# infil00p/openbts-ttsou

Measured on AMD Instinct MI355X. Metric: Mbursts/s (156.25-sym @ 4 sps) demod+detect, higher is better.
Workload: dtype f32

## Files before the change

### openbts-ttsou_amd/csrc/trxsig_corr.h

```cpp
#pragma once
#include "trxsig_dev.h"

namespace {

template <int SPS>
struct CorrGeom {
  static constexpr int NL = 36 * SPS;
  static constexpr int NC = (NL + 15) / 16;
  static constexpr int FRONT = 8 * SPS;
  static constexpr int WPAD0 = NC * 16 + 15 * SPS + 1;
  static constexpr int WPAD = ((WPAD0 + 15) / 32) * 32 + 16;
  static constexpr int H = (5 * SPS + 1 > 12) ? 5 * SPS + 1 : 12;
  static constexpr int NS = 2 * H + 1;
  static constexpr int NE = 20 * SPS;
  static constexpr int NEQ = (NE + 15) / 16;
  static constexpr int NPAIR = (NS + 2) / 2;
};
template <typename T>
__device__ __forceinline__ T &rec_slot(T *rec, int Bpad, int s, int b) { return rec[2 * ((size_t)(s >> 1) * Bpad + b) + (s & 1)]; }

template <int N>
__device__ __forceinline__ float add_row_shl(float acc, float v) {
  float r;
  if (N == 0) asm volatile("v_add_f32 %0, %1, %2" : "=v"(r) : "v"(v), "v"(acc));
  else asm volatile("v_add_f32_dpp %0, %1, %2 row_shl:%3 row_mask:0xf bank_mask:0xf bound_ctrl:1"
                    : "=v"(r) : "v"(v), "v"(acc), "n"(N));
  return r;
}
template <int SPS, int I>
__device__ __forceinline__ float energy_chain_step(float acc, const float (&nrm)[CorrGeom<SPS>::NEQ]) {
  if constexpr (I < CorrGeom<SPS>::NE) {
    acc = add_row_shl<I % 16>(acc, nrm[I / 16]);
    return energy_chain_step<SPS, I + 1>(acc, nrm);
  } else {
    return acc;
  }
}
template <int SPS, int I>
__device__ __forceinline__ float energy_chain(float acc, const float (&nrm)[CorrGeom<SPS>::NEQ]) {
  asm volatile("s_nop 1");
  return energy_chain_step<SPS, I>(acc, nrm);
}

template <int SPS>
struct CorrIn {
  typedef CorrGeom<SPS> G;
  static constexpr int NW = (CorrGeom<SPS>::NL + 15) / 16;
  cx w[NW];
  cx e[CorrGeom<SPS>::NEQ];
  int b;
  bool live, good;
  __device__ __forceinline__ void stage_window(cx *W, int r) const {
#pragma unroll
    for (int i = 0; i < NW; i++) {
      const int q = r + 16 * i;
      if (q < G::NL) W[G::FRONT + q] = w[i];
    }
  }
  __device__ __forceinline__ void stage_norms(float *ef, int r) const {
#pragma unroll
    for (int q = 0; q < G::NEQ; q++) {
      const int i = r + 16 * q;
      if (i < G::NE) ef[i] = norm2(e[q]);
    }
  }
};

template <int SPS>
__device__ __forceinline__ void corr_issue(CorrIn<SPS> &in, int b, int B, int r, const cx *__restrict__ samples,
                                           const int32_t *__restrict__ offset, const int32_t *__restrict__ length) {
  typedef CorrGeom<SPS> G;
  in.b = b;
  in.live = b < B;
  int off = 0, len = 0;
  if (in.live) { off = offset[b]; len = length[b]; }
  in.good = in.live && (off >= 0) && (len >= 92 * SPS) && (len <= 157 * SPS) && (len % SPS == 0);
  const cx *x = samples + (in.good ? off : 0);
#pragma unroll
  for (int i = 0; i < CorrIn<SPS>::NW; i++) {
    const int q = r + 16 * i;
    in.w[i] = (in.good && q < G::NL) ? x[56 * SPS + q] : mk(0, 0);
  }
#pragma unroll
  for (int q = 0; q < G::NEQ; q++) {
    const int i = r + 16 * q;
    in.e[q] = (in.good && i < G::NE) ? x[i] : mk(0, 0);
  }
}

template <int SPS, bool REC, bool EFIRST = false, unsigned TAPCLS = TRX_TAPS_GENERIC, typename IN = CorrIn<SPS>>
__device__ __forceinline__ void corr_round(const IN &in, cx *W, float4 *E, int lane, int r, const cx (&tap)[16],
                                           cx *__restrict__ rec, int Bpad, int &M_out, float &energy_out) {
  typedef CorrGeom<SPS> G;
  auto stage_norms = [&] { in.stage_norms(reinterpret_cast<float *>(E), r); };
  auto sum_norms = [&] {
    float energy = 0.0f;
#pragma unroll
    for (int i4 = 0; i4 < (G::NE + 3) / 4; i4++) {
      const float4 e = E[i4];
      energy = energy + e.x;
      if (4 * i4 + 1 < G::NE) energy = energy + e.y;
      if (4 * i4 + 2 < G::NE) energy = energy + e.z;
      if (4 * i4 + 3 < G::NE) energy = energy + e.w;
    }
    return energy;
  };
  float energy = 0.0f;
  if (EFIRST) {
    stage_norms();
    wave_lds_fence();
    energy = sum_norms();
    asm volatile("" : "+v"(energy));
    wave_lds_fence();
  }
  for (int q = r; q < G::FRONT; q += 16) W[q] = mk(0, 0);
  for (int q = G::FRONT + G::NL + r; q < G::WPAD; q += 16) W[q] = mk(0, 0);
  in.stage_window(W, r);
  if (!EFIRST) stage_norms();
  wave_lds_fence();
  if (!EFIRST) energy = sum_norms();

  float bestP = 0.0f;
  int bestT = -1;
  cx cval[G::NC];
  constexpr int CG = (SPS == 4) ? TRX_CORR_CG : 1;
  constexpr int UPC = 16 / SPS;
  constexpr int NU = UPC * (CG - 1) + 16;
#pragma unroll
  for (int c0 = 0; c0 < G::NC; c0 += CG) {
    cx sv[NU];
#pragma unroll
    for (int u = 0; u < NU; u++) sv[u] = W[r + 16 * c0 + SPS * u];
#pragma unroll
    for (int cc = 0; cc < CG; cc++) {
      if (c0 + cc < G::NC) {
        cx acc = mk(0, 0);
#pragma unroll
        for (int k = 15; k >= 0; k--) acc = cadd(acc, cmul_tap(sv[UPC * cc + k], tap[k], (TAPCLS >> (2 * k)) & 3));
        cval[c0 + cc] = acc;
      }
    }
  }
  wave_lds_fence();
#pragma unroll
  for (int c = 0; c < G::NC; c++) {
    const int t = r + 16 * c;
    if (t < G::NL) {
      W[t] = cval[c];
      const float p = norm2(cval[c]);
      if (p > bestP) { bestP = p; bestT = t; }
    }
  }
#pragma unroll
  for (int m = 1; m < 16; m <<= 1) {
    const float oP = __shfl_xor(bestP, m, 64);
    const int oT = __shfl_xor(bestT, m, 64);
    const bool take = (oP > bestP) || (oP == bestP && oT >= 0 && (bestT < 0 || oT < bestT));
    if (take) { bestP = oP; bestT = oT; }
  }
  wave_lds_fence();

  M_out = bestT;
  energy_out = energy;
  if (REC && in.live) {
    const int M = bestT;
    auto slot = [&](int s) {
      cx v = mk(0, 0);
      if (s < G::NS) {
        const int lag = M - G::H + s;
        if (lag >= 0 && lag < G::NL) v = W[lag];
      } else if (s == G::NS) {
        v = mk(__int_as_float(in.good ? M : -2), energy);
      }
      return v;
    };
    for (int j = r; j < G::NPAIR; j += 16) {
      const cx a = slot(2 * j), c = slot(2 * j + 1);
      reinterpret_cast<float4 *>(rec)[(size_t)j * Bpad + in.b] = make_float4(a.r, a.i, c.r, c.i);
    }
  }
  wave_lds_fence();
  (void)lane;
}


inline unsigned tap_classes(const TrxTables *hT, int tsc) {
  unsigned m = 0;
  for (int k = 0; k < 16; k++) {
    const trx_c32 a = hT->mid_ctap[tsc][k];
    const unsigned c = (a.r == 1.0f || a.r == -1.0f) ? 1u : ((a.i == 1.0f || a.i == -1.0f) ? 2u : 0u);
    m |= c << (2 * k);
  }
  return m;
}

}
```

### openbts-ttsou_amd/csrc/trxsig_dev.h

```cpp
#pragma once
#include <hip/hip_runtime.h>
#include <hip/hip_fp16.h>
#include <stdint.h>

#include <type_traits>

#include "trxsig_tables.h"
#include "trxsig_launch.h"

#ifndef TRX_CORR_CG
#define TRX_CORR_CG 3
#endif
#ifndef TRX_CORR_WPS
#define TRX_CORR_WPS 1
#endif
#ifndef TRX_CORR_ROUNDS
#define TRX_CORR_ROUNDS 1
#endif
#ifndef TRX_DEMOD_WAVES
#define TRX_DEMOD_WAVES 4
#endif

namespace {

typedef trx_c32 cx;

__device__ __forceinline__ cx mk(float r, float i) { cx z; z.r = r; z.i = i; return z; }
__device__ __forceinline__ cx cmul(cx x, cx a) { return mk(x.r * a.r - x.i * a.i, x.r * a.i + x.i * a.r); }
__device__ __forceinline__ cx cmulr(cx x, float a) { return mk(x.r * a, x.i * a); }
__device__ __forceinline__ cx cadd(cx x, cx a) { return mk(x.r + a.r, x.i + a.i); }
__device__ __forceinline__ float norm2(cx x) { return x.i * x.i + x.r * x.r; }
__device__ __forceinline__ cx cinv(cx x) { float n = norm2(x); return mk(x.r / n, -x.i / n); }
__device__ __forceinline__ cx cdiv(cx x, cx a) { return cmul(x, cinv(a)); }

template <int CTRL>
__device__ __forceinline__ float dpp_f(float v) {
  return __int_as_float(__builtin_amdgcn_update_dpp(0, __float_as_int(v), CTRL, 0xf, 0xf, true));
}
template <int CTRL>
__device__ __forceinline__ int dpp_i(int v) { return __builtin_amdgcn_update_dpp(0, v, CTRL, 0xf, 0xf, true); }
__device__ __forceinline__ float wave_sum_any_order(float v) {
  v += dpp_f<0xB1>(v);
  v += dpp_f<0x4E>(v);
  v += dpp_f<0x141>(v);
  v += dpp_f<0x140>(v);
  const float r0 = __int_as_float(__builtin_amdgcn_readlane(__float_as_int(v), 0));
  const float r1 = __int_as_float(__builtin_amdgcn_readlane(__float_as_int(v), 16));
  const float r2 = __int_as_float(__builtin_amdgcn_readlane(__float_as_int(v), 32));
  const float r3 = __int_as_float(__builtin_amdgcn_readlane(__float_as_int(v), 48));
  return ((r0 + r1) + r2) + r3;
}
__device__ __forceinline__ void argmax_take(float &P, int &T, float oP, int oT) {
  const bool take = (oP > P) || (oP == P && oT >= 0 && (T < 0 || oT < T));
  P = take ? oP : P;
  T = take ? oT : T;
}
__device__ __forceinline__ void wave_argmax(float &P, int &T) {
  argmax_take(P, T, dpp_f<0xB1>(P), dpp_i<0xB1>(T));
  argmax_take(P, T, dpp_f<0x4E>(P), dpp_i<0x4E>(T));
  argmax_take(P, T, dpp_f<0x141>(P), dpp_i<0x141>(T));
  argmax_take(P, T, dpp_f<0x140>(P), dpp_i<0x140>(T));
  float bp = __int_as_float(__builtin_amdgcn_readlane(__float_as_int(P), 0));
  int bt = __builtin_amdgcn_readlane(T, 0);
#pragma unroll
  for (int r = 16; r < 64; r += 16)
    argmax_take(bp, bt, __int_as_float(__builtin_amdgcn_readlane(__float_as_int(P), r)), __builtin_amdgcn_readlane(T, r));
  P = bp; T = bt;
}

typedef float v2f __attribute__((ext_vector_type(2)));
__device__ __forceinline__ v2f pk(cx z) { v2f v = {z.r, z.i}; return v; }
__device__ __forceinline__ v2f pk_cmul(v2f x, v2f a) {
  v2f p, q, r;
  asm("v_pk_mul_f32 %0, %1, %2 op_sel_hi:[0,1]" : "=v"(p) : "v"(x), "v"(a));
  asm("v_pk_mul_f32 %0, %1, %2 op_sel:[1,1] op_sel_hi:[1,0]" : "=v"(q) : "v"(x), "v"(a));
  asm("v_pk_add_f32 %0, %1, %2 neg_lo:[0,1]" : "=v"(r) : "v"(p), "v"(q));
  return r;
}
__device__ __forceinline__ v2f pk_mul(v2f x, v2f a) {
  v2f r;
  asm("v_pk_mul_f32 %0, %1, %2" : "=v"(r) : "v"(x), "v"(a));
  return r;
}
template <int HI>
__device__ __forceinline__ v2f pk_mul_tap(v2f x, v2f t) {
  v2f r;
  if (HI) asm("v_pk_mul_f32 %0, %1, %2 op_sel:[0,1] op_sel_hi:[1,1]" : "=v"(r) : "v"(x), "v"(t));
  else asm("v_pk_mul_f32 %0, %1, %2 op_sel_hi:[1,0]" : "=v"(r) : "v"(x), "v"(t));
  return r;
}
__device__ __forceinline__ v2f pk_csub(v2f x, v2f a) {
  v2f r;
  asm("v_pk_add_f32 %0, %1, %2 neg_lo:[0,1] neg_hi:[0,1]" : "=v"(r) : "v"(x), "v"(a));
  return r;
}
__device__ __forceinline__ cx unpk(v2f v) { return mk(v.x, v.y); }
__device__ __forceinline__ v2f pk_cadd(v2f x, v2f a) {
  v2f r;
  asm("v_pk_add_f32 %0, %1, %2" : "=v"(r) : "v"(x), "v"(a));
  return r;
}

struct SmpC32 {
  static constexpr int kBytes = 8;
  static __device__ __forceinline__ cx ld(const void *base, long long i) { return reinterpret_cast<const cx *>(base)[i]; }
  typedef cx raw_t;
  static __device__ __forceinline__ raw_t ldraw(const void *base, long long i) { return reinterpret_cast<const cx *>(base)[i]; }
  static __device__ __forceinline__ raw_t zero() { return mk(0, 0); }
  static __device__ __forceinline__ cx widen(raw_t r) { return r; }
  static __device__ __forceinline__ float4 ld2(const void *base, long long first, int q) {
    return reinterpret_cast<const float4 *>(reinterpret_cast<const cx *>(base) + first)[q];
  }
};
struct SmpF16 {
  static constexpr int kBytes = 4;
  static __device__ __forceinline__ cx ld(const void *base, long long i) {
    const float2 v = __half22float2(reinterpret_cast<const __half2 *>(base)[i]);
    return mk(v.x, v.y);
  }
  typedef unsigned raw_t;
  static __device__ __forceinline__ raw_t ldraw(const void *base, long long i) { return reinterpret_cast<const unsigned *>(base)[i]; }
  static __device__ __forceinline__ raw_t zero() { return 0u; }
  static __device__ __forceinline__ cx widen(raw_t r) {
    const float2 v = __half22float2(*reinterpret_cast<const __half2 *>(&r));
    return mk(v.x, v.y);
  }
  static __device__ __forceinline__ float4 ld2(const void *base, long long first, int q) {
    const uint2 u = reinterpret_cast<const uint2 *>(reinterpret_cast<const __half2 *>(base) + first)[q];
    const float2 a = __half22float2(*reinterpret_cast<const __half2 *>(&u.x)), b = __half22float2(*reinterpret_cast<const __half2 *>(&u.y));
    return make_float4(a.x, a.y, b.x, b.y);
  }
};

struct TapArg { float v[32]; };

#define TRX_TAPS_GENERIC 0u
template <int SPS> struct TapPattern {
  static constexpr unsigned value = (SPS == 4) ? 0x19999999u : 0x99999999u;
};
__device__ __forceinline__ float fma_steer(float a, float b, float c) {
  float r;
  asm("v_fma_f32 %0, %1, %2, %3 ; steering" : "=v"(r) : "v"(a), "v"(b), "v"(c));
  return r;
}
__device__ __forceinline__ float fma_steer_s(float a, float b_sgpr, float c) {
  float r;
  asm("v_fma_f32 %0, %1, %2, %3 ; steering" : "=v"(r) : "v"(a), "s"(b_sgpr), "v"(c));
  return r;
}
__device__ __forceinline__ cx cmul_tap(cx x, cx a, int cls) {
  if (cls == 1) {
    const float p = x.i * a.i, q = x.r * a.i;
    cx z;
    asm("v_fma_f32 %0, %2, %4, -%5 ; exact-product\n\tv_fma_f32 %1, %3, %4, %6 ; exact-product"
        : "=&v"(z.r), "=v"(z.i) : "v"(x.r), "v"(x.i), "s"(a.r), "v"(p), "v"(q));
    return z;
  }
  if (cls == 2) {
    const float p = x.r * a.r, q = x.i * a.r;
    cx z;
    asm("v_fma_f32 %0, %3, -%4, %5 ; exact-product\n\tv_fma_f32 %1, %2, %4, %6 ; exact-product"
        : "=&v"(z.r), "=v"(z.i) : "v"(x.r), "v"(x.i), "s"(a.i), "v"(p), "v"(q));
    return z;
  }
  return cmul(x, a);
}

// ... 49 lines not shown
```

### openbts-ttsou_amd/csrc/trxsig_normal.hip

```cpp
#include "trxsig_bisect.h"
#include "trxsig_corr.h"
#include "trxsig_demod.h"
#include "trxsig_rxgen.h"

#ifndef TRX_RXC_WPS
#define TRX_RXC_WPS 1
#endif
#ifndef TRX_RXD_WPS
#define TRX_RXD_WPS 1
#endif

namespace {

template <int SPS, unsigned TAPCLS>
__global__ __launch_bounds__(256, TRX_CORR_WPS) void k_tsc_corr(const TrxTables *__restrict__ T,
                                                  const cx *__restrict__ samples,
                                                  const int32_t *__restrict__ offset,
                                                  const int32_t *__restrict__ length, int B, TapArg taps,
                                                  cx *__restrict__ rec, int Bpad) {
  typedef CorrGeom<SPS> G;
  static_assert(8 * G::WPAD >= 4 * G::NE, "the energy norms are staged in the row itself");
  __shared__ __attribute__((aligned(16))) cx rows[16][G::WPAD];
  (void)T;
  const int lane = threadIdx.x & 63, wave = threadIdx.x >> 6;
  const int row = lane >> 4, r = lane & 15;
  const int slot = wave * 4 + row;

  cx tap[16];
#pragma unroll
  for (int k = 0; k < 16; k++) tap[k] = mk(taps.v[2 * k], taps.v[2 * k + 1]);

  typedef CorrIn<SPS> In;
  In in[TRX_CORR_ROUNDS];
#pragma unroll
  for (int i = 0; i < TRX_CORR_ROUNDS; i++)
    corr_issue<SPS>(in[i], (blockIdx.x * TRX_CORR_ROUNDS + i) * 16 + slot, B, r, samples, offset, length);
#pragma unroll
  for (int i = 0; i < TRX_CORR_ROUNDS; i++) {
    int M;
    float energy;
    corr_round<SPS, true, true, TAPCLS, In>(in[i], rows[slot], reinterpret_cast<float4 *>(rows[slot]), lane, r, tap, rec, Bpad, M, energy);
  }
}


#ifdef TRX_TUNING_BUILD
template <int SPS>
__global__ __launch_bounds__(64) void k_tsc_peak(const TrxTables *__restrict__ T,
                                                 const cx *__restrict__ rec, int Bpad, int B, int tsc,
                                                 float detect_thresh, float energy_thresh,
                                                 uint8_t *__restrict__ flags, cx *__restrict__ amp_out,
                                                 float *__restrict__ toa_out,
                                                 float *__restrict__ avgpwr_out) {
  typedef CorrGeom<SPS> G;
  __shared__ cx loc[26][64];
  __shared__ float pw[G::NS][64];
  const int lane = threadIdx.x;
  const int b = blockIdx.x * 64 + lane;
  const bool live = b < B;
  const int bb = live ? b : B - 1;

  const cx meta = rec_slot(rec, Bpad, G::NS, bb);
  const int M = __float_as_int(meta.r);
  const float energy = meta.i;
  const bool good = M != -2;
#pragma unroll
  for (int s = 0; s < G::NS; s++) {
    const cx v = rec_slot(rec, Bpad, s, bb);
    pw[s][lane] = norm2(v);
    const int j = s - (G::H - 12);
    if (j >= 0 && j < 24) {
      const int lag = M - 12 + j;
      loc[j][lane] = (lag > G::NL - 2) ? mk(0, 0) : v;
    }
  }
  loc[24][lane] = mk(0, 0);
  loc[25][lane] = mk(0, 0);

  float peakIx;
  const cx peak = peak_bisect<64>(T->sinc_grid, loc, lane, M, &peakIx);

  float toa = peakIx;
  cx amp = peak;
  bool detected = false;
  const bool energy_ok = good && (energy_thresh < 0.0f ||
                                  energy / (float)(unsigned)G::NE > energy_thresh * energy_thresh);
  if (!(toa < 0.0f) && !(toa > (float)G::NL) && good) {
    const int p = (int)rintf(toa);
    float valley = 0.0f;
    int numRms = 0;
#pragma unroll
    for (int i = 2 * SPS; i <= 5 * SPS; i++) {
      const int lo = p - i, hi = p + i;
      int slo = lo - M + G::H, shi = hi - M + G::H;
      slo = slo < 0 ? 0 : slo; shi = shi > G::NS - 1 ? G::NS - 1 : shi;
      const float vlo = pw[slo][lane], vhi = pw[shi][lane];
      if (lo >= 0) { valley += vlo; numRms++; }
      if (hi < G::NL) { valley += vhi; numRms++; }
    }
    if (numRms < 2) {
      amp = mk(0, 0);
    } else {
      const float RMS = (float)((double)sqrtf(valley / (float)numRms) + 0.00001);
      const float peakToMean = sqrtf(norm2(amp)) / RMS;
      amp = cdiv(amp, T->mid_gain[tsc]);
      toa = toa - T->mid_toa[tsc];
      toa = toa - (float)((66 - 56) * SPS);
      detected = peakToMean > detect_thresh;
    }
  } else {
    amp = mk(0, 0);
  }
  if (!energy_ok) { amp = mk(0, 0); toa = 0.0f; detected = false; }

  if (live) {
    uint8_t fl = 0;
    if (!good) fl = TRXSIG_F_BADLEN;
    else fl = (energy_ok ? TRXSIG_F_ENERGY : 0) | (detected ? TRXSIG_F_DETECT : 0);
    flags[b] = fl;
    amp_out[b] = amp;
    toa_out[b] = toa;
    if (avgpwr_out) avgpwr_out[b] = good ? energy / (float)(unsigned)G::NE : 0.0f;
  }
}


template <int SPS>
struct Peak8Geom {
  typedef CorrGeom<SPS> G;
  static constexpr int NV = 2 * (3 * SPS + 1);
  static constexpr int O_PW = 26 * 2;
  static constexpr int O_V = O_PW + ((G::NS + 3) & ~3);
  static constexpr int STRIDE = O_V + ((NV + 3) & ~3);
};

template <int SPS>
__global__ __launch_bounds__(256, 8) void k_tsc_peak8(const TrxTables *__restrict__ T, const cx *__restrict__ rec, int Bpad,
                                                   int B, cx gain_inv, float mid_toa, float detect_thresh,
                                                   float energy_thresh, uint8_t *__restrict__ flags,
                                                   cx *__restrict__ amp_out, float *__restrict__ toa_out,
                                                   float *__restrict__ avgpwr_out) {
  typedef CorrGeom<SPS> G;
  typedef Peak8Geom<SPS> P8;
  __shared__ __attribute__((aligned(16))) float stab[32][24];
  __shared__ __attribute__((aligned(16))) float scratch[32][P8::STRIDE];
  {
    float tv[3];
#pragma unroll
    for (int k = 0; k < 3; k++) { const int ix = threadIdx.x * 3 + k; tv[k] = T->sinc_grid[16 * (ix / 24)][ix % 24]; }
#pragma unroll
    for (int k = 0; k < 3; k++) { const int ix = threadIdx.x * 3 + k; stab[ix / 24][ix % 24] = tv[k]; }
  }
  const int lane = threadIdx.x & 63;
  const int r = lane & 7;
  const int slot = threadIdx.x >> 3;
  const int b = blockIdx.x * 32 + slot;
  const bool live = b < B;
  const int bb = live ? b : B - 1;
  float *S = scratch[slot];
  cx *loc = reinterpret_cast<cx *>(S);
  float *pw = S + P8::O_PW, *V = S + P8::O_V;

  const cx meta = rec_slot(rec, Bpad, G::NS, bb);
  const int M = __float_as_int(meta.r);
  const float energy = meta.i;
  const bool good = M != -2;
#pragma unroll
  for (int s0 = 0; s0 < G::NS; s0 += 8) {
    const int sl = s0 + r;
    if (sl < G::NS) {
      const cx v = rec_slot(rec, Bpad, sl, bb);
      pw[sl] = norm2(v);
      const int j = sl - (G::H - 12);
      if (j >= 0 && j < 24) loc[j] = (M - 12 + j > G::NL - 2) ? mk(0, 0) : v;
    }
  }
  if (r < 2) loc[24 + r] = mk(0, 0);
  __syncthreads();

  int e = 0;
  asm volatile("" : "+v"(e));
  bool active = true;
  cx peak = mk(0, 0);
  {
    const int rel2 = kFusedRel2.v[r], rel1 = kFusedRel1.v[r];
#pragma unroll
    for (int st = 0; st < 4; st++) {
      const int inc_last = 128 >> (2 * st);
      const int el = e + (rel2 >> 2) * inc_last;
      float srow[24];
      if (st < 3) {
        const float4 *rw = reinterpret_cast<const float4 *>(stab[(el & 511) >> 4]);
#pragma unroll
        for (int q = 0; q < 6; q++) {
          const float4 t4 = rw[q];
          srow[4 * q] = t4.x; srow[4 * q + 1] = t4.y; srow[4 * q + 2] = t4.z; srow[4 * q + 3] = t4.w;
        }
      } else {
        fused_row(T, el, srow);
      }
      const cx pt = fused_point(loc, el, rel2 & 3, srow);
      fused_decide<8, 2, false>(pt, lane, 2 * inc_last, e, active, peak);
    }
    {
      float srow[24];
      fused_row(T, e, srow);
      const cx pt = fused_point(loc, e, rel1 & 3, srow);
      fused_decide<8, 1, false>(pt, lane, 1, e, active, peak);
    }
    float srow[24];
    fused_row(T, e, srow);
    peak = fused_point(loc, e, 1, srow);
    asm volatile("" : "+v"(peak.r), "+v"(peak.i));
  }
  cx amp;
  float toa;
  bool detected, energy_ok;
  fused_tail<SPS, 8>([&](int lag) { const int sl = lag - M + G::H; return (sl < 0 || sl >= G::NS) ? 0.0f : pw[sl]; }, V, r, M, e,
                     peak, good, energy, gain_inv, mid_toa, detect_thresh, energy_thresh, amp, toa, detected, energy_ok);
  if (live && r == 0) {
    uint8_t fl = 0;
    if (!good) fl = TRXSIG_F_BADLEN;
    else fl = (energy_ok ? TRXSIG_F_ENERGY : 0) | (detected ? TRXSIG_F_DETECT : 0);
    flags[b] = fl;
    amp_out[b] = amp;
    toa_out[b] = toa;
    if (avgpwr_out) avgpwr_out[b] = good ? energy / (float)(unsigned)G::NE : 0.0f;
  }
}



#endif

#ifndef TRX_PEAK2_THREADS
#define TRX_PEAK2_THREADS 512
#endif
constexpr int kPeak2Threads = TRX_PEAK2_THREADS;
template <int SPS>
__global__ __launch_bounds__(kPeak2Threads) void k_tsc_peak2(const TrxTables *__restrict__ T, const cx *__restrict__ rec, int Bpad,
                                                   int B, cx gain_inv, float mid_toa, float detect_thresh,
                                                   float energy_thresh, uint8_t *__restrict__ flags,
                                                   cx *__restrict__ amp_out, float *__restrict__ toa_out,
                                                   float *__restrict__ avgpwr_out) {
  typedef CorrGeom<SPS> G;
  constexpr int NL = G::NL, NE = G::NE, NP = 3 * SPS + 3;
  __shared__ __attribute__((aligned(16))) SincLds stab;
  const int tid = threadIdx.x;
  const int h = tid & 1;
  const int b = blockIdx.x * (kPeak2Threads / 2) + (tid >> 1);
  const bool live = b < B;
  const int bb = live ? b : B - 1;
#ifdef TRX_PEAK_PROBE
  long long pt_[16] = {0};
  int pk_ = 0;
#define TRX_STAMP() pt_[pk_++] = clock64()
#else
#define TRX_STAMP()
#endif
  TRX_STAMP();

  float4 tv[3072 / kPeak2Threads];
  sinc_lds_issue<kPeak2Threads>(T, tid, tv);
  const cx meta = rec_slot(rec, Bpad, G::NS, bb);
  const int M = __float_as_int(meta.r);
  const float energy = meta.i;
  const bool good = M != -2;
  const float4 *rec4 = reinterpret_cast<const float4 *>(rec);
  cx q[23];
  {
    constexpr int S0 = G::H - 12, P0 = S0 >> 1;
    float4 pw[12];
#pragma unroll
    for (int i = 0; i < 12; i++) pw[i] = rec4[(size_t)(P0 + h + i) * Bpad + bb];
#pragma unroll
    for (int k = 0; k < 23; k++) {
      const int ix = k + 2 * h;
      const float4 p4 = pw[((S0 + k) >> 1) - P0];
      const cx v = ((S0 + k) & 1) ? mk(p4.z, p4.w) : mk(p4.x, p4.y);
      q[k] = (M - 12 + ix > NL - 2) ? mk(0, 0) : v;
    }
  }
  cx vmine_[NP];
  constexpr int VLO = G::H - (5 * SPS + 1), VHI = G::H + (2 * SPS - 1);
  if constexpr ((VLO & 1) == 0 && (VHI & 1) == 0) {
    float4 pv[(NP + 1) / 2];
#pragma unroll
    for (int i = 0; i < (NP + 1) / 2; i++) pv[i] = rec4[(size_t)(((h ? VHI : VLO) >> 1) + i) * Bpad + bb];
#pragma unroll
    for (int k = 0; k < NP; k++) vmine_[k] = (k & 1) ? mk(pv[k >> 1].z, pv[k >> 1].w) : mk(pv[k >> 1].x, pv[k >> 1].y);
  } else {
#pragma unroll
    for (int k = 0; k < NP; k++) vmine_[k] = rec_slot(rec, Bpad, (h ? VHI : VLO) + k, bb);
  }
  sinc_lds_store<kPeak2Threads>(stab, tid, tv);
  TRX_STAMP();
  __syncthreads();
  TRX_STAMP();

  int e;
  const cx peak = pair_bisect(stab, q, h, e);
  TRX_STAMP();
  const float early = (float)(M - 1) + (float)e * 0.001953125f;
  float toa = early + 1.0f;
  cx amp = peak;
  bool detected = false;
  const bool energy_ok = good && (energy_thresh < 0.0f || energy / (float)(unsigned)NE > energy_thresh * energy_thresh);
  const bool sane = !(toa < 0.0f) && !(toa > (float)NL) && good;
  if (sane) {
    const int pk = (int)rintf(toa);
    const int a = pk - M + 1;
    float plo[NP], phi[NP];
#pragma unroll
    for (int k = 0; k < NP; k++) {
      const float mine = norm2(vmine_[k]);
      const float other = __int_as_float(__builtin_amdgcn_update_dpp(0, __float_as_int(mine), 0xB1, 0xf, 0xf, true));
      plo[k] = h ? other : mine; phi[k] = h ? mine : other;
    }
    float valley = 0.0f;
#pragma unroll
    for (int i = 2 * SPS; i <= 5 * SPS; i++) {
      const int t = 5 * SPS - i, u = i - 2 * SPS;
      const float vlo = a == 0 ? plo[t] : (a == 1 ? plo[t + 1] : plo[t + 2]);
      const float vhi = a == 0 ? phi[u] : (a == 1 ? phi[u + 1] : phi[u + 2]);
      valley = valley + vlo;
      valley = valley + vhi;
    }
    int nlo = (pk < 5 * SPS ? pk : 5 * SPS) - 2 * SPS + 1;
    int nhi = (NL - 1 - pk < 5 * SPS ? NL - 1 - pk : 5 * SPS) - 2 * SPS + 1;
    nlo = nlo < 0 ? 0 : nlo; nhi = nhi < 0 ? 0 : nhi;
    const int numRms = nlo + nhi;
    if (numRms < 2) {
      amp = mk(0, 0);
    } else {
      const float RMS = (float)((double)sqrtf(valley / (float)numRms) + 0.00001);
      const float peakToMean = sqrtf(norm2(amp)) / RMS;
      amp = cmul(amp, gain_inv);
      toa = toa - mid_toa;
      toa = toa - (float)((66 - 56) * SPS);
      detected = peakToMean > detect_thresh;
    }
  } else {
    amp = mk(0, 0);
  }
  if (!energy_ok) { amp = mk(0, 0); toa = 0.0f; detected = false; }

  if (live && h == 0) {
    uint8_t fl = 0;
    if (!good) fl = TRXSIG_F_BADLEN;
    else fl = (energy_ok ? TRXSIG_F_ENERGY : 0) | (detected ? TRXSIG_F_DETECT : 0);
    flags[b] = fl;
    amp_out[b] = amp;
    toa_out[b] = toa;
    if (avgpwr_out) avgpwr_out[b] = good ? energy / (float)(unsigned)G::NE : 0.0f;
  }
#ifdef TRX_PEAK_PROBE
  TRX_STAMP();
  if (live && avgpwr_out) {
    long long v = 0;
    for (int k = 1; k < 16; k++) if ((b & 15) == k) v = pt_[k] - pt_[0];
    if (h == 0) avgpwr_out[b] = (float)v;
  }
#endif
#undef TRX_STAMP
}

template <int SPS, unsigned TAPCLS>
__global__ __launch_bounds__(256, TRX_RXC_WPS) void k_tsc_corr_rx(TrxRxGen a, int B, TapArg taps, cx *__restrict__ rec, int Bpad) {
  static_assert(SPS == 4, "the fused front end is the 260 : 96 resampler");
  typedef CorrGeom<SPS> G;
  constexpr int XCAP = 160;
  static_assert(G::WPAD >= XCAP, "the raw stretch is parked in the burst's own row");
  __shared__ __attribute__((aligned(16))) cx rows[16][G::WPAD];
  __shared__ float4 tpb_s[RXG_NT];
  if (threadIdx.x < RXG_NT) tpb_s[threadIdx.x] = a.tpb[threadIdx.x];
  __syncthreads();
  const int lane = threadIdx.x & 63, wave = threadIdx.x >> 6;
  const int row = lane >> 4, r = lane & 15;
  const int slot = wave * 4 + row;
  cx tap[16];
#pragma unroll
  for (int k = 0; k < 16; k++) tap[k] = mk(taps.v[2 * k], taps.v[2 * k + 1]);
  const int b = blockIdx.x * 16 + slot;
  CorrIn<SPS> in;
  in.b = b; in.live = b < B; in.good = in.live;
  const RxBurst u = rx_burst(a, in.live ? b : 0);
  const int jlo = rx_index(u.g0, a.skipD).j0 - 3;
  cx *X = rows[slot];
  {
    short2 v[XCAP / 16];
#pragma unroll
    for (int i = 0; i < XCAP / 16; i++) v[i] = rx_raw(a, u.s, jlo + r + 16 * i);
#pragma unroll
    for (int i = 0; i < XCAP / 16; i++) X[r + 16 * i] = rx_widen(a, v[i]);
  }
  wave_lds_fence();
  {
    static_assert(G::NL % 16 == 0 && G::NE % 16 == 0, "every lane owns a sample in every round");
    const int nb = rx_boundary(u.g0);
    RxIdx ix = rx_index(u.g0 + 56 * SPS + r, a.skipD);
#pragma unroll
    for (int i = 0; i < CorrIn<SPS>::NW; i++) {
      in.w[i] = rx_sample(X, tpb_s, jlo, ix, nb - (56 * SPS + r + 16 * i), a.w0, a.w1);
      ix = rx_step<16>(ix);
      if (i % 3 == 2) asm volatile("" : "+v"(in.w[i].r), "+v"(in.w[i].i), "+v"(in.w[i - 1].r), "+v"(in.w[i - 1].i), "+v"(in.w[i - 2].r), "+v"(in.w[i - 2].i) : : "memory");
    }
    ix = rx_index(u.g0 + r, a.skipD);
#pragma unroll
    for (int q = 0; q < G::NEQ; q++) {
      in.e[q] = rx_sample(X, tpb_s, jlo, ix, nb - (r + 16 * q), a.w0, a.w1);
      ix = rx_step<16>(ix);
      if (q % 3 == 2) asm volatile("" : "+v"(in.e[q].r), "+v"(in.e[q].i), "+v"(in.e[q - 1].r), "+v"(in.e[q - 1].i), "+v"(in.e[q - 2].r), "+v"(in.e[q - 2].i) : : "memory");
    }
  }
  wave_lds_fence();
  int M;
  float energy;
  corr_round<SPS, true, true, TAPCLS>(in, rows[slot], reinterpret_cast<float4 *>(rows[slot]), lane, r, tap, rec, Bpad, M, energy);
}

template <int SPS, bool TOL = false>
__global__ __launch_bounds__(64 * TRX_DEMOD_WAVES, TRX_RXD_WPS) void k_demod_rx(const TrxTables *__restrict__ T, TrxRxGen a, int B,
                                                                  const cx *__restrict__ amp_in, const float *__restrict__ toa_in,
                                                                  const uint8_t *__restrict__ flags, int need_mask,
                                                                  float *__restrict__ soft, uint8_t *__restrict__ hard, int nsoft,
                                                                  int stride) {
  static_assert(SPS == 4, "the fused front end is the 260 : 96 resampler");
  typedef DemodGeom<SPS, 148> G;
  constexpr int XCAP = 256;
  static_assert(G::U >= XCAP, "the raw stretch is parked in the burst's staging area");
  __shared__ cx ph[TRX_DEMOD_WAVES][G::U];
  __shared__ float4 tpb_s[RXG_NT];
  if (threadIdx.x < RXG_NT) tpb_s[threadIdx.x] = a.tpb[threadIdx.x];
  __syncthreads();
  const int lane = threadIdx.x & 63;
  const int wave = __builtin_amdgcn_readfirstlane(threadIdx.x >> 6);
  const int b = blockIdx.x * TRX_DEMOD_WAVES + wave;
  if (b >= B) return;
  float *sb = soft + (size_t)b * stride;
  uint8_t *hb = hard ? hard + (size_t)b * stride : nullptr;
  const cx amp = amp_in[b];
  const float toa = toa_in[b];
  bool enabled = fabsf(toa) <= 4096.0f;
  if (flags) enabled = enabled && (need_mask ? ((flags[b] & need_mask) == need_mask) : (flags[b] != 0));
  if (!enabled) {
    for (int m = lane; m < nsoft; m += 64) { sb[m] = 0.0f; if (hb) hb[m] = 0; }
    return;
  }
  const RxBurst u = rx_burst(a, b);
  const int jlo = rx_index(u.g0, a.skipD).j0 - 3;
  cx *X = ph[wave];
  {
    short2 v[XCAP / 64];
#pragma unroll
    for (int i = 0; i < XCAP / 64; i++) v[i] = rx_raw(a, u.s, jlo + lane + 64 * i);
#pragma unroll
    for (int i = 0; i < XCAP / 64; i++) X[lane + 64 * i] = rx_widen(a, v[i]);
  }
  wave_lds_fence();
  constexpr int NSL = (157 * SPS + 63) / 64;
  cx sv[NSL];
  {
    const int nb = rx_boundary(u.g0);
    RxIdx ix = rx_index(u.g0 + lane, a.skipD);
#pragma unroll
    for (int i = 0; i < NSL; i++) {
      sv[i] = rx_sample(X, tpb_s, jlo, ix, nb - (lane + 64 * i), a.w0, a.w1);
      ix = rx_step<64>(ix);
      if (i % 2 == 1) asm volatile("" : "+v"(sv[i].r), "+v"(sv[i].i), "+v"(sv[i - 1].r), "+v"(sv[i - 1].i) : : "memory");
    }
  }
  const int N = u.N;
  auto stage = [&](cx *P, cx inv, int lo) {
    typedef DemodGeom<SPS, 148> D;
    const int u0 = lane + lo;
    if (u0 >= 0) {
      cx *p0 = P + (u0 % SPS) * D::QLEN + u0 / SPS;
#pragma unroll
      for (int i = 0; i < NSL; i++)
        if (lane + 64 * i < N && u0 + 64 * i < D::U) p0[i * (64 / SPS)] = cmul(sv[i], inv);
// ... 190 lines not shown
```

Before: 636.1.

## Use tight unpadded LDS rows for SPS=4 correlation and raise occupancy

For SPS=4 the correlation kernel now stores each burst window in a tight LDS row without zero-padded front/back slack. Out-of-window taps are skipped at compile time or masked per lane, so the padding-zeroing stores go away. The smaller shared footprint, together with a column group of 1 and a launch-bounds occupancy hint of 8, is meant to fit more waves per CU. The cost is extra masking branches at the window edges, and register pressure may now be limited by the occupancy hint.

```diff
diff --git a/openbts-ttsou_amd/csrc/trxsig_corr.h b/openbts-ttsou_amd/csrc/trxsig_corr.h
--- a/openbts-ttsou_amd/csrc/trxsig_corr.h
+++ b/openbts-ttsou_amd/csrc/trxsig_corr.h
@@ -16,6 +16,23 @@
   static constexpr int NEQ = (NE + 15) / 16;
   static constexpr int NPAIR = (NS + 2) / 2;
 };
+template <int SPS, bool TIGHT>
+struct CorrRow {
+  typedef CorrGeom<SPS> G;
+  static constexpr int FRONT = TIGHT ? 0 : G::FRONT;
+  static constexpr int STRIDE = TIGHT ? G::NL : G::WPAD;
+  static constexpr int GUARD = TIGHT ? 16 : 0;
+  static_assert(!TIGHT || G::NL % 16 == 0, "a tight row has no slack behind the window");
+  static_assert((2 * STRIDE) % 64 == 32, "rows 32 dwords apart (mod 64)");
+  static_assert(8 * STRIDE >= 4 * G::NE, "the energy norms are staged in the row itself");
+};
+template <int SPS, bool TIGHT, int NROWS>
+struct CorrRows {
+  typedef CorrRow<SPS, TIGHT> R;
+  __attribute__((aligned(16))) cx w[2 * R::GUARD + NROWS * R::STRIDE];
+  static_assert(R::GUARD % 2 == 0, "rows stay 16-byte aligned");
+  __device__ __forceinline__ cx *row(int slot) { return w + R::GUARD + slot * R::STRIDE; }
+};
 template <typename T>
 __device__ __forceinline__ T &rec_slot(T *rec, int Bpad, int s, int b) { return rec[2 * ((size_t)(s >> 1) * Bpad + b) + (s & 1)]; }
 
@@ -54,7 +71,7 @@
 #pragma unroll
     for (int i = 0; i < NW; i++) {
       const int q = r + 16 * i;
-      if (q < G::NL) W[G::FRONT + q] = w[i];
+      if (q < G::NL) W[q] = w[i];
     }
   }
   __device__ __forceinline__ void stage_norms(float *ef, int r) const {
@@ -88,10 +105,11 @@
   }
 }
 
-template <int SPS, bool REC, bool EFIRST = false, unsigned TAPCLS = TRX_TAPS_GENERIC, typename IN = CorrIn<SPS>>
+template <int SPS, bool REC, bool EFIRST = false, unsigned TAPCLS = TRX_TAPS_GENERIC, typename IN = CorrIn<SPS>, bool TIGHT = false>
 __device__ __forceinline__ void corr_round(const IN &in, cx *W, float4 *E, int lane, int r, const cx (&tap)[16],
                                            cx *__restrict__ rec, int Bpad, int &M_out, float &energy_out) {
   typedef CorrGeom<SPS> G;
+  typedef CorrRow<SPS, TIGHT> R;
   auto stage_norms = [&] { in.stage_norms(reinterpret_cast<float *>(E), r); };
   auto sum_norms = [&] {
     float energy = 0.0f;
@@ -113,9 +131,11 @@
     asm volatile("" : "+v"(energy));
     wave_lds_fence();
   }
-  for (int q = r; q < G::FRONT; q += 16) W[q] = mk(0, 0);
-  for (int q = G::FRONT + G::NL + r; q < G::WPAD; q += 16) W[q] = mk(0, 0);
-  in.stage_window(W, r);
+  if (!TIGHT) {
+    for (int q = r; q < G::FRONT; q += 16) W[q] = mk(0, 0);
+    for (int q = G::FRONT + G::NL + r; q < G::WPAD; q += 16) W[q] = mk(0, 0);
+  }
+  in.stage_window(W + R::FRONT, r);
   if (!EFIRST) stage_norms();
   wave_lds_fence();
   if (!EFIRST) energy = sum_norms();
@@ -128,15 +148,27 @@
   constexpr int NU = UPC * (CG - 1) + 16;
 #pragma unroll
   for (int c0 = 0; c0 < G::NC; c0 += CG) {
+    auto q0 = [&](int u) { return 16 * c0 + SPS * u - 8 * SPS; };
+    auto absent = [&](int u) { return TIGHT && (q0(u) + 15 < 0 || q0(u) >= G::NL); };
     cx sv[NU];
 #pragma unroll
-    for (int u = 0; u < NU; u++) sv[u] = W[r + 16 * c0 + SPS * u];
+    for (int u = 0; u < NU; u++) {
+      if (absent(u)) { sv[u] = mk(0, 0); continue; }
+      sv[u] = W[R::FRONT + r + q0(u)];
+      if (TIGHT && (q0(u) < 0 || q0(u) + 15 >= G::NL)) {
+        const int q = r + q0(u);
+        if (q < 0 || q >= G::NL) sv[u] = mk(0, 0);
+      }
+    }
 #pragma unroll
     for (int cc = 0; cc < CG; cc++) {
       if (c0 + cc < G::NC) {
         cx acc = mk(0, 0);
 #pragma unroll
-        for (int k = 15; k >= 0; k--) acc = cadd(acc, cmul_tap(sv[UPC * cc + k], tap[k], (TAPCLS >> (2 * k)) & 3));
+        for (int k = 15; k >= 0; k--) {
+          if (absent(UPC * cc + k)) continue;
+          acc = cadd(acc, cmul_tap(sv[UPC * cc + k], tap[k], (TAPCLS >> (2 * k)) & 3));
+        }
         cval[c0 + cc] = acc;
       }
     }
diff --git a/openbts-ttsou_amd/csrc/trxsig_dev.h b/openbts-ttsou_amd/csrc/trxsig_dev.h
--- a/openbts-ttsou_amd/csrc/trxsig_dev.h
+++ b/openbts-ttsou_amd/csrc/trxsig_dev.h
@@ -9,10 +9,10 @@
 #include "trxsig_launch.h"
 
 #ifndef TRX_CORR_CG
-#define TRX_CORR_CG 3
+#define TRX_CORR_CG 1
 #endif
 #ifndef TRX_CORR_WPS
-#define TRX_CORR_WPS 1
+#define TRX_CORR_WPS 8
 #endif
 #ifndef TRX_CORR_ROUNDS
 #define TRX_CORR_ROUNDS 1
diff --git a/openbts-ttsou_amd/csrc/trxsig_normal.hip b/openbts-ttsou_amd/csrc/trxsig_normal.hip
--- a/openbts-ttsou_amd/csrc/trxsig_normal.hip
+++ b/openbts-ttsou_amd/csrc/trxsig_normal.hip
@@ -13,14 +13,13 @@
 namespace {
 
 template <int SPS, unsigned TAPCLS>
-__global__ __launch_bounds__(256, TRX_CORR_WPS) void k_tsc_corr(const TrxTables *__restrict__ T,
+__global__ __launch_bounds__(256, SPS == 4 ? TRX_CORR_WPS : 1) void k_tsc_corr(const TrxTables *__restrict__ T,
                                                   const cx *__restrict__ samples,
                                                   const int32_t *__restrict__ offset,
                                                   const int32_t *__restrict__ length, int B, TapArg taps,
                                                   cx *__restrict__ rec, int Bpad) {
-  typedef CorrGeom<SPS> G;
-  static_assert(8 * G::WPAD >= 4 * G::NE, "the energy norms are staged in the row itself");
-  __shared__ __attribute__((aligned(16))) cx rows[16][G::WPAD];
+  constexpr bool TIGHT = SPS == 4;
+  __shared__ CorrRows<SPS, TIGHT, 16> rows;
   (void)T;
   const int lane = threadIdx.x & 63, wave = threadIdx.x >> 6;
   const int row = lane >> 4, r = lane & 15;
@@ -39,7 +38,7 @@
   for (int i = 0; i < TRX_CORR_ROUNDS; i++) {
     int M;
     float energy;
-    corr_round<SPS, true, true, TAPCLS, In>(in[i], rows[slot], reinterpret_cast<float4 *>(rows[slot]), lane, r, tap, rec, Bpad, M, energy);
+    corr_round<SPS, true, true, TAPCLS, In, TIGHT>(in[i], rows.row(slot), reinterpret_cast<float4 *>(rows.row(slot)), lane, r, tap, rec, Bpad, M, energy);
   }
 }
 
```

Measured after the change: 640.6, median of 4. No clear change (+0.7%).

## Precompute valley power sums in correlation kernel, shrink record passed to peak kernels

Applied to the files above, without the earlier changes.

The correlation kernel now computes the three candidate valley sums (one per possible peak offset) from the correlation row in LDS and stores them with the meta slot. The record written per burst shrinks from the wide ±H window to 25 correlation taps plus sums. The peak kernels no longer load and square the wide window or reduce valley powers. This cuts global traffic and register pressure in the peak stage, at the cost of extra LDS work and fences in the correlation kernel.

```diff
diff --git a/openbts-ttsou_amd/csrc/trxsig_corr.h b/openbts-ttsou_amd/csrc/trxsig_corr.h
--- a/openbts-ttsou_amd/csrc/trxsig_corr.h
+++ b/openbts-ttsou_amd/csrc/trxsig_corr.h
@@ -10,11 +10,15 @@
   static constexpr int FRONT = 8 * SPS;
   static constexpr int WPAD0 = NC * 16 + 15 * SPS + 1;
   static constexpr int WPAD = ((WPAD0 + 15) / 32) * 32 + 16;
-  static constexpr int H = (5 * SPS + 1 > 12) ? 5 * SPS + 1 : 12;
-  static constexpr int NS = 2 * H + 1;
   static constexpr int NE = 20 * SPS;
   static constexpr int NEQ = (NE + 15) / 16;
-  static constexpr int NPAIR = (NS + 2) / 2;
+  static constexpr int RH = 12;
+  static constexpr int NRC = 2 * RH + 1;
+  static constexpr int NP = 3 * SPS + 3;
+  static constexpr int S_VS = NRC, S_META = NRC + 2;
+  static constexpr int NPAIR = (NRC + 3) / 2;
+  static_assert(2 * (WPAD - NL) >= 2 * NP + 4, "the valley powers and sums are parked behind the correlation in the row");
+  static_assert(NP <= 16, "a lane of the row per valley power");
 };
 template <typename T>
 __device__ __forceinline__ T &rec_slot(T *rec, int Bpad, int s, int b) { return rec[2 * ((size_t)(s >> 1) * Bpad + b) + (s & 1)]; }
@@ -164,19 +168,31 @@
   energy_out = energy;
   if (REC && in.live) {
     const int M = bestT;
-    auto slot = [&](int s) {
-      cx v = mk(0, 0);
-      if (s < G::NS) {
-        const int lag = M - G::H + s;
-        if (lag >= 0 && lag < G::NL) v = W[lag];
-      } else if (s == G::NS) {
-        v = mk(__int_as_float(in.good ? M : -2), energy);
+    auto corr_at = [&](int lag) { return (lag >= 0 && lag < G::NL) ? W[lag] : mk(0, 0); };
+    float *P = reinterpret_cast<float *>(W + G::NL);
+    if (r < G::NP) {
+      P[r] = norm2(corr_at(M - 1 - 5 * SPS + r));
+      P[G::NP + r] = norm2(corr_at(M - 1 + 2 * SPS + r));
+    }
+    wave_lds_fence();
+    if (r < 3) {
+      float vs = 0.0f;
+#pragma unroll
+      for (int i = 2 * SPS; i <= 5 * SPS; i++) {
+        vs = vs + P[5 * SPS - i + r];
+        vs = vs + P[G::NP + i - 2 * SPS + r];
       }
-      return v;
-    };
-    for (int j = r; j < G::NPAIR; j += 16) {
-      const cx a = slot(2 * j), c = slot(2 * j + 1);
-      reinterpret_cast<float4 *>(rec)[(size_t)j * Bpad + in.b] = make_float4(a.r, a.i, c.r, c.i);
+      P[2 * G::NP + r] = vs;
+    }
+    wave_lds_fence();
+    if (r < G::NPAIR) {
+      cx a = corr_at(M - G::RH + 2 * r), c = corr_at(M - G::RH + 2 * r + 1);
+      if (2 * r + 1 == G::S_VS) c = mk(P[2 * G::NP], P[2 * G::NP + 1]);
+      if (2 * r == G::S_VS + 1) {
+        a = mk(P[2 * G::NP + 2], energy);
+        c = mk(__int_as_float(in.good ? M : -2), 0.0f);
+      }
+      reinterpret_cast<float4 *>(rec)[(size_t)r * Bpad + in.b] = make_float4(a.r, a.i, c.r, c.i);
     }
   }
   wave_lds_fence();
diff --git a/openbts-ttsou_amd/csrc/trxsig_normal.hip b/openbts-ttsou_amd/csrc/trxsig_normal.hip
--- a/openbts-ttsou_amd/csrc/trxsig_normal.hip
+++ b/openbts-ttsou_amd/csrc/trxsig_normal.hip
@@ -54,25 +54,20 @@
                                                  float *__restrict__ avgpwr_out) {
   typedef CorrGeom<SPS> G;
   __shared__ cx loc[26][64];
-  __shared__ float pw[G::NS][64];
   const int lane = threadIdx.x;
   const int b = blockIdx.x * 64 + lane;
   const bool live = b < B;
   const int bb = live ? b : B - 1;
 
-  const cx meta = rec_slot(rec, Bpad, G::NS, bb);
-  const int M = __float_as_int(meta.r);
-  const float energy = meta.i;
+  const int M = __float_as_int(rec_slot(rec, Bpad, G::S_META, bb).r);
+  const cx vs01 = rec_slot(rec, Bpad, G::S_VS, bb), vs2e = rec_slot(rec, Bpad, G::S_VS + 1, bb);
+  const float energy = vs2e.i;
   const bool good = M != -2;
 #pragma unroll
-  for (int s = 0; s < G::NS; s++) {
-    const cx v = rec_slot(rec, Bpad, s, bb);
-    pw[s][lane] = norm2(v);
-    const int j = s - (G::H - 12);
-    if (j >= 0 && j < 24) {
-      const int lag = M - 12 + j;
-      loc[j][lane] = (lag > G::NL - 2) ? mk(0, 0) : v;
-    }
+  for (int j = 0; j < 24; j++) {
+    const cx v = rec_slot(rec, Bpad, j, bb);
+    const int lag = M - 12 + j;
+    loc[j][lane] = (lag > G::NL - 2) ? mk(0, 0) : v;
   }
   loc[24][lane] = mk(0, 0);
   loc[25][lane] = mk(0, 0);
@@ -87,16 +82,13 @@
                                   energy / (float)(unsigned)G::NE > energy_thresh * energy_thresh);
   if (!(toa < 0.0f) && !(toa > (float)G::NL) && good) {
     const int p = (int)rintf(toa);
-    float valley = 0.0f;
+    const int a = p - M + 1;
+    const float valley = a == 0 ? vs01.r : (a == 1 ? vs01.i : vs2e.r);
     int numRms = 0;
 #pragma unroll
     for (int i = 2 * SPS; i <= 5 * SPS; i++) {
-      const int lo = p - i, hi = p + i;
-      int slo = lo - M + G::H, shi = hi - M + G::H;
-      slo = slo < 0 ? 0 : slo; shi = shi > G::NS - 1 ? G::NS - 1 : shi;
-      const float vlo = pw[slo][lane], vhi = pw[shi][lane];
-      if (lo >= 0) { valley += vlo; numRms++; }
-      if (hi < G::NL) { valley += vhi; numRms++; }
+      if (p - i >= 0) numRms++;
+      if (p + i < G::NL) numRms++;
     }
     if (numRms < 2) {
       amp = mk(0, 0);
@@ -129,8 +121,7 @@
 struct Peak8Geom {
   typedef CorrGeom<SPS> G;
   static constexpr int NV = 2 * (3 * SPS + 1);
-  static constexpr int O_PW = 26 * 2;
-  static constexpr int O_V = O_PW + ((G::NS + 3) & ~3);
+  static constexpr int O_V = 26 * 2;
   static constexpr int STRIDE = O_V + ((NV + 3) & ~3);
 };
 
@@ -159,21 +150,17 @@
   const int bb = live ? b : B - 1;
   float *S = scratch[slot];
   cx *loc = reinterpret_cast<cx *>(S);
-  float *pw = S + P8::O_PW, *V = S + P8::O_V;
-
-  const cx meta = rec_slot(rec, Bpad, G::NS, bb);
-  const int M = __float_as_int(meta.r);
-  const float energy = meta.i;
+  float *V = S + P8::O_V;
+
+  const int M = __float_as_int(rec_slot(rec, Bpad, G::S_META, bb).r);
+  const cx vs01 = rec_slot(rec, Bpad, G::S_VS, bb), vs2e = rec_slot(rec, Bpad, G::S_VS + 1, bb);
+  const float energy = vs2e.i;
   const bool good = M != -2;
 #pragma unroll
-  for (int s0 = 0; s0 < G::NS; s0 += 8) {
-    const int sl = s0 + r;
-    if (sl < G::NS) {
-      const cx v = rec_slot(rec, Bpad, sl, bb);
-      pw[sl] = norm2(v);
-      const int j = sl - (G::H - 12);
-      if (j >= 0 && j < 24) loc[j] = (M - 12 + j > G::NL - 2) ? mk(0, 0) : v;
-    }
+  for (int j0 = 0; j0 < 24; j0 += 8) {
+    const int j = j0 + r;
+    const cx v = rec_slot(rec, Bpad, j, bb);
+    loc[j] = (M - 12 + j > G::NL - 2) ? mk(0, 0) : v;
   }
   if (r < 2) loc[24 + r] = mk(0, 0);
   __syncthreads();
@@ -216,8 +203,10 @@
   cx amp;
   float toa;
   bool detected, energy_ok;
-  fused_tail<SPS, 8>([&](int lag) { const int sl = lag - M + G::H; return (sl < 0 || sl >= G::NS) ? 0.0f : pw[sl]; }, V, r, M, e,
-                     peak, good, energy, gain_inv, mid_toa, detect_thresh, energy_thresh, amp, toa, detected, energy_ok);
+  const int pk = (int)rintf((float)(M - 1) + (float)e * 0.001953125f + 1.0f);
+  const float valley = pk == M - 1 ? vs01.r : (pk == M ? vs01.i : vs2e.r);
+  fused_tail<SPS, 8>([&](int lag) { return lag == pk - 2 * SPS ? valley : 0.0f; }, V, r, M, e, peak, good, energy, gain_inv, mid_toa,
+                     detect_thresh, energy_thresh, amp, toa, detected, energy_ok);
   if (live && r == 0) {
     uint8_t fl = 0;
     if (!good) fl = TRXSIG_F_BADLEN;
@@ -244,7 +233,7 @@
                                                    cx *__restrict__ amp_out, float *__restrict__ toa_out,
                                                    float *__restrict__ avgpwr_out) {
   typedef CorrGeom<SPS> G;
-  constexpr int NL = G::NL, NE = G::NE, NP = 3 * SPS + 3;
+  constexpr int NL = G::NL, NE = G::NE;
   __shared__ __attribute__((aligned(16))) SincLds stab;
   const int tid = threadIdx.x;
   const int h = tid & 1;
@@ -262,36 +251,23 @@
 
   float4 tv[3072 / kPeak2Threads];
   sinc_lds_issue<kPeak2Threads>(T, tid, tv);
-  const cx meta = rec_slot(rec, Bpad, G::NS, bb);
-  const int M = __float_as_int(meta.r);
-  const float energy = meta.i;
+  const float4 *rec4 = reinterpret_cast<const float4 *>(rec);
+  const float4 p12 = rec4[(size_t)12 * Bpad + bb], p13 = rec4[(size_t)13 * Bpad + bb];
+  const int M = __float_as_int(p13.z);
+  const float energy = p13.y;
   const bool good = M != -2;
-  const float4 *rec4 = reinterpret_cast<const float4 *>(rec);
   cx q[23];
   {
-    constexpr int S0 = G::H - 12, P0 = S0 >> 1;
     float4 pw[12];
 #pragma unroll
-    for (int i = 0; i < 12; i++) pw[i] = rec4[(size_t)(P0 + h + i) * Bpad + bb];
+    for (int i = 0; i < 12; i++) pw[i] = rec4[(size_t)(h + i) * Bpad + bb];
 #pragma unroll
     for (int k = 0; k < 23; k++) {
       const int ix = k + 2 * h;
-      const float4 p4 = pw[((S0 + k) >> 1) - P0];
-      const cx v = ((S0 + k) & 1) ? mk(p4.z, p4.w) : mk(p4.x, p4.y);
+      const float4 p4 = pw[k >> 1];
+      const cx v = (k & 1) ? mk(p4.z, p4.w) : mk(p4.x, p4.y);
       q[k] = (M - 12 + ix > NL - 2) ? mk(0, 0) : v;
     }
-  }
-  cx vmine_[NP];
-  constexpr int VLO = G::H - (5 * SPS + 1), VHI = G::H + (2 * SPS - 1);
-  if constexpr ((VLO & 1) == 0 && (VHI & 1) == 0) {
-    float4 pv[(NP + 1) / 2];
-#pragma unroll
-    for (int i = 0; i < (NP + 1) / 2; i++) pv[i] = rec4[(size_t)(((h ? VHI : VLO) >> 1) + i) * Bpad + bb];
-#pragma unroll
-    for (int k = 0; k < NP; k++) vmine_[k] = (k & 1) ? mk(pv[k >> 1].z, pv[k >> 1].w) : mk(pv[k >> 1].x, pv[k >> 1].y);
-  } else {
-#pragma unroll
-    for (int k = 0; k < NP; k++) vmine_[k] = rec_slot(rec, Bpad, (h ? VHI : VLO) + k, bb);
   }
   sinc_lds_store<kPeak2Threads>(stab, tid, tv);
   TRX_STAMP();
@@ -310,22 +286,7 @@
   if (sane) {
     const int pk = (int)rintf(toa);
     const int a = pk - M + 1;
-    float plo[NP], phi[NP];
-#pragma unroll
-    for (int k = 0; k < NP; k++) {
-      const float mine = norm2(vmine_[k]);
-      const float other = __int_as_float(__builtin_amdgcn_update_dpp(0, __float_as_int(mine), 0xB1, 0xf, 0xf, true));
-      plo[k] = h ? other : mine; phi[k] = h ? mine : other;
-    }
-    float valley = 0.0f;
-#pragma unroll
-    for (int i = 2 * SPS; i <= 5 * SPS; i++) {
-      const int t = 5 * SPS - i, u = i - 2 * SPS;
-      const float vlo = a == 0 ? plo[t] : (a == 1 ? plo[t + 1] : plo[t + 2]);
-      const float vhi = a == 0 ? phi[u] : (a == 1 ? phi[u + 1] : phi[u + 2]);
-      valley = valley + vlo;
-      valley = valley + vhi;
-    }
+    const float valley = a == 0 ? p12.z : (a == 1 ? p12.w : p13.x);
     int nlo = (pk < 5 * SPS ? pk : 5 * SPS) - 2 * SPS + 1;
     int nhi = (NL - 1 - pk < 5 * SPS ? NL - 1 - pk : 5 * SPS) - 2 * SPS + 1;
     nlo = nlo < 0 ? 0 : nlo; nhi = nhi < 0 ? 0 : nhi;
```

Measured after the change: 633.1 before, 635.3 after, median of 5. No clear change (+0.3%).
